# hrz2000/CustomNeRF

Hardware: AMD Instinct MI355X
Metric: training rays/s (higher is better)
Workload: dtype f16

## Files before the change

customnerf_amd/_lib.py:

```python
import ctypes as C
import os

import torch

_HERE = os.path.dirname(os.path.abspath(__file__))
LIB_PATH = os.path.join(_HERE, "libcustomnerf_hip.so")
ABI_VERSION = 7

vp, u32, u64, f32, i32 = C.c_void_p, C.c_uint32, C.c_uint64, C.c_float, C.c_int

SIGNATURES = {
    "cnerf_abi_version": [],
    "cnerf_profile_stage_events": [vp, u32],
    "cnerf_near_far_from_aabb": [vp, vp, vp, u32, f32, vp, vp, vp],
    "cnerf_sph_from_ray": [vp, vp, f32, u32, vp, vp],
    "cnerf_morton3D": [vp, u32, vp, vp],
    "cnerf_morton3D_invert": [vp, u32, vp, vp],
    "cnerf_packbits": [vp, u32, f32, vp, vp],
    "cnerf_march_rays_train": [vp, vp, vp, f32, f32, u32, u32, u32, u32, u32, vp, vp, vp, vp, vp, vp, vp, vp, vp],
    "cnerf_march_rays_train_count": [vp, vp, vp, f32, f32, u32, u32, u32, u32, vp, vp, vp, vp, vp, vp],
    "cnerf_march_rays_train_write": [vp, vp, vp, f32, f32, u32, u32, u32, u32, u32, vp, vp, vp, vp, vp, vp, vp, vp],
    "cnerf_march_rays_train_count_hits": [vp, vp, vp, f32, f32, u32, u32, u32, u32, vp, vp, vp, vp, vp, vp, vp],
    "cnerf_march_rays_train_write_hits": [vp, vp, f32, f32, u32, u32, u32, u32, u32, vp, vp, vp, vp, vp, vp, vp, vp],
    "cnerf_composite_rays_train_forward": [vp, vp, vp, vp, u32, u32, f32, vp, vp, vp, u32, vp],
# ... 9 lines not shown
    "cnerf_grid_encode_backward_prepared": [vp, vp, vp, vp, u32, u32, u32, u32, u32, f32, u32, u32, i32, u32, i32, vp, u64, vp],
    "cnerf_grid_encode_backward_workspace_bytes": [vp, u32, u32, u32, u32, u32, f32, u32, i32, vp],
    "cnerf_grid_encode_backward_needs_plan": [vp, u32, u32, u32, u32, u32, f32, u32, u32, i32, vp],
    "cnerf_grad_total_variation": [vp, vp, vp, vp, f32, u32, u32, u32, u32, f32, u32, u32, i32, vp],
    "cnerf_cast_f32_to_f16": [vp, vp, u64, vp],
    "cnerf_field_forward": [vp, vp, vp, u32, u32, u32, u32, u32, vp, vp, vp, vp, vp, i32, vp],
    "cnerf_field_forward_strided": [vp, vp, vp, u32, u32, u32, u32, u32, vp, vp, vp, vp, vp, i32, u32, vp],
    "cnerf_field_backward": [vp, vp, vp, u32, u32, u32, u32, u32, vp, vp, vp, vp, vp, vp, vp, vp, vp, vp, u64, i32, vp],
    "cnerf_field_backward_ex": [vp, vp, vp, u32, u32, u32, u32, u32, vp, vp, vp, vp, vp, vp, vp, vp, vp, vp, u64, i32, vp, vp],
    "cnerf_field_backward_workspace_bytes": [u32, u32, u32, u32, i32, vp],
    "cnerf_stream_capture_id": [vp, vp],
    "cnerf_field_weight_image_bytes": [u32, u32, u32, vp],
    "cnerf_field_pack_weights": [u32, u32, u32, vp, vp, vp, vp, u64, vp],
    "cnerf_field_forward_img": [vp, vp, vp, u32, u32, u32, u32, u32, vp, vp, vp, vp, vp, i32, u32, vp, vp],
    "cnerf_field_backward_img": [vp, vp, vp, u32, u32, u32, u32, u32, vp, vp, vp, vp, vp, vp, vp, vp, vp, vp, u64, i32, vp, vp, vp],
    "cnerf_mlp_forward": [vp, u32, vp, u32, u32, u32, u32, u32, i32, vp, u32, i32, vp],
    "cnerf_mlp_backward": [vp, u32, vp, vp, u32, u32, u32, u32, u32, u32, i32, vp, u32, vp, vp, u64, i32, vp],
    "cnerf_mlp_backward_workspace_bytes": [u32, u32, u32, u32, u32, i32, vp],
    "cnerf_generate_rays": [vp, u32, u32, u32, f32, f32, f32, f32, f32, i32, vp, vp, vp],
    "cnerf_generate_rays_fisheye": [vp, u32, u32, u32, f32, f32, f32, f32, f32, vp, vp, vp, vp],
    "cnerf_occupancy_points": [vp, u32, f32, f32, vp, vp],
    "cnerf_occupancy_update": [vp, u32, f32, vp, vp, vp],
    "cnerf_occupancy_finalize_pack": [vp, u32, f32, vp, u32, vp, vp, vp],
    "cnerf_sample_pdf": [vp, vp, vp, u32, u32, u32, vp, vp],
    "cnerf_sample_coarse": [vp, vp, vp, vp, vp, vp, u32, u32, vp, vp, vp],
    "cnerf_sample_fine_merge": [vp, vp, vp, vp, vp, vp, vp, vp, u32, u32, u32, vp, vp, vp],
    "cnerf_sample_fine_merge_split": [vp, vp, vp, vp, vp, vp, vp, vp, u32, u32, u32, vp, vp, vp, vp, vp],
    "cnerf_sample_coarse_unit": [vp, vp, vp, vp, vp, vp, u32, u32, vp, vp, vp, f32, vp],
    "cnerf_sample_fine_merge_split_unit": [vp, vp, vp, vp, vp, vp, vp, vp, u32, u32, u32, vp, vp, vp, vp, f32, vp],
    "cnerf_composite_run": [vp, vp, vp, vp, vp, u32, u32, u32, i32, f32, vp, vp, vp],
# ... 242 lines not shown
```

customnerf_amd/csrc/field_bwd.hip:

```cpp
#include "field_bwd_common.h"
#include "field_dw.h"

struct FieldWs {
    uint32_t enc, h1, h2, fea, hd, hr, dir, z1, z2, z3, zd, zdo, zr, zro, rows;
};
__host__ __device__ __forceinline__ FieldWs fb_ws_layout(const FieldDims &d) {
    FieldWs w;
    uint32_t o = 0;
    w.enc = o; o += d.enc_pad;
    w.h1 = o; o += 64;
    w.h2 = o; o += (d.n_hidden_geo == 2) ? 64 : 0;
    w.fea = o; o += 64;
    w.hd = o; o += 64;
    w.hr = o; o += 64;
    w.dir = o; o += 32;
    w.z1 = o; o += 64;
    w.z2 = o; o += (d.n_hidden_geo == 2) ? 64 : 0;
    w.z3 = o; o += 64;
    w.zd = o; o += 64;
    w.zdo = o; o += 8;
    w.zr = o; o += 64;
    w.zro = o; o += 8;
    w.rows = o;
    return w;
// ... 221 lines not shown
    fb_add_job(pl, wo.zro, dm.n_rgb_out, wo.hr, 64, 2, FLD_HID * in_r0, 64, 0, 16);
    const uint32_t splits = fb_dw_splits(n_tiles, pl.k_tiles_per_split);
    float *partials = reinterpret_cast<float *>(reinterpret_cast<unsigned char *>(workspace) + fb_part_off(dm, P_, H ? CNERF_F16 : CNERF_F32));
    hipLaunchKernelGGL((k_field_bwd_dw<H>), dim3(pl.n_tiles, splits), dim3(FLD_THREADS), 0, st, workspace, ld, n_tiles, pl, g_net, g_den, g_rgb, partials);
    rc = cn_launch_status();
    if (rc) return rc;
    ff_reduce_partials(partials, splits, po.total, po.d0, po.r0 - po.d0, g_net, g_den, g_rgb, st);
    return cn_launch_status();
}

static bool fb_use_fused(const FieldDims &dm, int dtype) {
    static const int env = cn_tune_env("CNERF_FIELD_FUSED_BWD", 1);
    return env && dtype == CNERF_F16 && dm.enc_pad <= 32;
}

extern "C" {

int cnerf_field_backward_workspace_bytes(uint32_t P_, uint32_t enc_dim, uint32_t n_hidden_geo, uint32_t n_rgb_out, int dtype, uint64_t *bytes) {
    if (!bytes) return CNERF_ENULL;
    FieldDims dm;
    int rc = fld_dims(enc_dim, n_hidden_geo, n_rgb_out, dm);
    if (rc) return rc;
    if (dtype != CNERF_F32 && dtype != CNERF_F16) return CNERF_EINVAL;
    if (fb_use_fused(dm, dtype)) *bytes = ff_workspace_bytes(dm);
    else *bytes = fb_workspace_bytes(dm, P_, dtype);
    return CNERF_OK;
}

int cnerf_field_backward(const void *enc, const float *xyz, const float *dirs, uint32_t dir_group, uint32_t P_, uint32_t enc_dim,
                         uint32_t n_hidden_geo, uint32_t n_rgb_out, const float *params_net, const float *params_den, const float *params_rgb,
                         const float *grad_sigma, const float *grad_rgbc, void *grad_enc, float *grad_params_net, float *grad_params_den,
// ... 3 lines not shown
}

int cnerf_field_backward_ex(const void *enc, const float *xyz, const float *dirs, uint32_t dir_group, uint32_t P_, uint32_t enc_dim,
                            uint32_t n_hidden_geo, uint32_t n_rgb_out, const float *params_net, const float *params_den, const float *params_rgb,
                            const float *grad_sigma, const float *grad_rgbc, void *grad_enc, float *grad_params_net, float *grad_params_den,
                            float *grad_params_rgb, void *workspace, uint64_t workspace_bytes, int dtype, const uint8_t *tile_live, void *stream) {
    return cnerf_field_backward_img(enc, xyz, dirs, dir_group, P_, enc_dim, n_hidden_geo, n_rgb_out, params_net, params_den, params_rgb, grad_sigma, grad_rgbc,
                                    grad_enc, grad_params_net, grad_params_den, grad_params_rgb, workspace, workspace_bytes, dtype, tile_live, nullptr, stream);
}

int cnerf_field_backward_img(const void *enc, const float *xyz, const float *dirs, uint32_t dir_group, uint32_t P_, uint32_t enc_dim,
                             uint32_t n_hidden_geo, uint32_t n_rgb_out, const float *params_net, const float *params_den, const float *params_rgb,
                             const float *grad_sigma, const float *grad_rgbc, void *grad_enc, float *grad_params_net, float *grad_params_den,
                             float *grad_params_rgb, void *workspace, uint64_t workspace_bytes, int dtype, const uint8_t *tile_live,
                             const void *weight_image, void *stream) {
    FieldDims dm;
    int rc = fld_dims(enc_dim, n_hidden_geo, n_rgb_out, dm);
    if (rc) return rc;
    if (dtype != CNERF_F32 && dtype != CNERF_F16) return CNERF_EINVAL;
    if (P_ == 0) return CNERF_OK;
    if (!enc || !xyz || !dirs || !params_net || !params_den || !params_rgb || !grad_sigma || !grad_rgbc || !grad_enc || !grad_params_net ||
        !grad_params_den || !grad_params_rgb || !workspace)
        return CNERF_ENULL;
    if (dir_group == 0 || (((uintptr_t)grad_rgbc) & 15) || (((uintptr_t)workspace) & 15) || (((uintptr_t)weight_image) & 15)) return CNERF_EINVAL;
    uint64_t need = 0;
    cnerf_field_backward_workspace_bytes(P_, enc_dim, n_hidden_geo, n_rgb_out, dtype, &need);
    if (workspace_bytes < need) return CNERF_EINVAL;
    if (fb_use_fused(dm, dtype))
        return ff_launch(enc, xyz, dirs, dir_group, P_, dm, params_net, params_den, params_rgb, grad_sigma, grad_rgbc, grad_enc, grad_params_net,
                         grad_params_den, grad_params_rgb, workspace, tile_live, CN_STREAM(stream), weight_image);
    if (dtype == CNERF_F16)
        return fb_launch<true>(enc, xyz, dirs, dir_group, P_, dm, params_net, params_den, params_rgb, grad_sigma, grad_rgbc, grad_enc,
                               grad_params_net, grad_params_den, grad_params_rgb, workspace, CN_STREAM(stream));
    return fb_launch<false>(enc, xyz, dirs, dir_group, P_, dm, params_net, params_den, params_rgb, grad_sigma, grad_rgbc, grad_enc, grad_params_net,
                            grad_params_den, grad_params_rgb, workspace, CN_STREAM(stream));
}

}
```

customnerf_amd/csrc/field_bwd_common.h:

```cpp
#pragma once
#include "field_common.h"


template <bool H, int T, int NS>
__device__ __forceinline__ void fb_gemm(const typename Prec<H>::elem_t *wf, uint32_t S, uint32_t s0, const typename Prec<H>::frag_t *b, uint32_t lane,
                                        cn_f16v (&acc)[T]) {
    asm volatile("" ::: "memory");
    fld_gemm<H, T, NS>(wf, S, s0, b, lane, acc);
}

template <bool H>
__device__ __forceinline__ void fb_stage_layer_T(typename Prec<H>::elem_t *dst, const float *__restrict__ W, uint32_t rows, uint32_t in_stride,
                                                 uint32_t col0, uint32_t n_in, uint32_t T, uint32_t S) {
    using P = Prec<H>;
    const uint32_t total = T * S * 64 * P::J;
    for (uint32_t i = threadIdx.x; i < total; i += blockDim.x) {
        const uint32_t j = i % P::J, lane = (i / P::J) % 64, ts = i / (P::J * 64);
        const uint32_t s = ts % S, t = ts / S;
        const uint32_t col = 32 * t + (lane & 31), hi = lane >> 5;
        const uint32_t row = (uint32_t)fld_col_clayout<H>(s, hi, j);
        float v = 0.0f;
        if (row < rows && col < n_in) v = W[(size_t)row * in_stride + col0 + col];
        dst[i] = (typename P::elem_t)v;
    }
// ... 139 lines not shown
    o.n1 = p; p += (dm.n_hidden_geo == 2) ? 4096 : 0;
    o.n2 = p; p += 4096;
    o.d0 = p; p += 4096;
    o.dO = p; p += 16 * 64;
    o.r0 = p; p += 64 * 96;
    o.rO = p; p += 16 * 64;
    o.total = p;
    return o;
}

void ff_reduce_partials(const float *partials, uint32_t n_partials, uint32_t total, uint32_t n_net, uint32_t n_den, float *g_net, float *g_den, float *g_rgb,
                        hipStream_t st);
uint64_t ff_workspace_bytes(const FieldDims &dm);
int ff_launch(const void *enc, const float *xyz, const float *dirs, uint32_t dir_group, uint32_t P_, const FieldDims &dm, const float *pnet,
              const float *pden, const float *prgb, const float *g_sigma, const float *g_rgbc, void *grad_enc, float *g_net, float *g_den,
              float *g_rgb, void *workspace, const uint8_t *tile_live, hipStream_t st, const void *wimg);
bool x2_eligible(const FieldDims &dm);
int x2_launch(const void *enc, const float *xyz, const float *dirs, uint32_t dir_group, uint32_t P_, const FieldDims &dm, const float *pnet, const float *pden,
              const float *prgb, const float *g_sigma, const float *g_rgbc, void *grad_enc, float *g_net, float *g_den, float *g_rgb, void *workspace,
              uint32_t max_partials, const uint8_t *tile_live, hipStream_t st, const void *wimg);
```

customnerf_amd/csrc/field_bwd_fused.hip:

```cpp
#include "field_bwd_common.h"

#define FF_ROWB 256
#define FF_ROWS 256
#define FF_STAGE_BYTES (FF_ROWB * FF_ROWS)
#define FF_PIN(col, hi) asm volatile("" : "+v"(col), "+v"(hi)::"memory")

__device__ __forceinline__ void ff_put(unsigned char *st, uint32_t row, uint32_t col, _Float16 v) {
    *reinterpret_cast<_Float16 *>(st + row * FF_ROWB + (((col >> 3) ^ (row & 15)) << 4) + ((col & 7) << 1)) = v;
}
__device__ __forceinline__ cn_h8 ff_frag(const unsigned char *st, uint32_t row, uint32_t s, uint32_t hi) {
    return *reinterpret_cast<const cn_h8 *>(st + row * FF_ROWB + ((((2 * s + hi)) ^ (row & 15)) << 4));
}
__device__ __forceinline__ void ff_stage_clayout(unsigned char *st, uint32_t row0, uint32_t col, uint32_t hi, const cn_h8 *b) {
#pragma unroll
    for (int s = 0; s < 4; s++) {
        asm volatile("" : "+v"(col), "+v"(hi)::"memory");
#pragma unroll
        for (int j = 0; j < 8; j++) ff_put(st, row0 + (uint32_t)fld_col_clayout<true>(s, hi, j), col, b[s][j]);
    }
}
template <int NS>
__device__ __forceinline__ void ff_stage_natural(unsigned char *st, uint32_t row0, uint32_t col, uint32_t hi, const cn_h8 *b) {
#pragma unroll
    for (int s = 0; s < NS; s++) {
// ... 300 lines not shown
        *dst = gn;
        if (!(fabsf(gn) <= 3.4e38f) && found_inf) *found_inf = 1.0f;
    }
}

#define FF_MAX_BLOCKS 512
uint64_t ff_workspace_bytes(const FieldDims &dm) { return (uint64_t)FF_MAX_BLOCKS * ff_offsets(dm).total * sizeof(float) + 256; }

void ff_reduce_partials(const float *partials, uint32_t n_partials, uint32_t total, uint32_t n_net, uint32_t n_den, float *g_net, float *g_den, float *g_rgb,
                        hipStream_t st) {
    hipLaunchKernelGGL(k_field_reduce_partials, dim3(cn_div_up(total, 64)), dim3(256), 0, st, partials, n_partials, total, n_net, n_den, g_net, g_den, g_rgb, g_cn_found_inf);
}

int ff_launch(const void *enc, const float *xyz, const float *dirs, uint32_t dir_group, uint32_t P_, const FieldDims &dm, const float *pnet,
              const float *pden, const float *prgb, const float *g_sigma, const float *g_rgbc, void *grad_enc, float *g_net, float *g_den,
              float *g_rgb, void *workspace, const uint8_t *tile_live, hipStream_t st, const void *wimg) {
    if (x2_eligible(dm)) {
        return x2_launch(enc, xyz, dirs, dir_group, P_, dm, pnet, pden, prgb, g_sigma, g_rgbc, grad_enc, g_net, g_den, g_rgb, workspace, FF_MAX_BLOCKS, tile_live, st,
                         wimg);
    }
    (void)wimg;
    const FieldLds lo = fld_lds_layout<true>(dm);
    const FieldLdsT lt = fb_ldsT_layout<true>(dm);
    const uint32_t lds_bytes = (lo.off[7] + lt.off[7]) * sizeof(_Float16) + FF_STAGE_BYTES;
    if (lds_bytes > 160 * 1024) return CNERF_EINVAL;
    const uint32_t n_tiles = cn_div_up(P_, FLD_TILE);
    uint32_t blocks = cn_div_up(n_tiles, FLD_WAVES);
    if (blocks > 256) blocks = 256;
    const FfOff po = ff_offsets(dm);
    float *partials = reinterpret_cast<float *>(workspace);
    hipError_t e = hipMemsetAsync(partials, 0, (size_t)blocks * po.total * sizeof(float), st);
    if (e != hipSuccess) return (int)e;
    const bool ok = fld_dispatch(dm, [&](auto se16, auto ng) {
        auto kern = k_field_bwd_fused<se16, ng, (se16 + 1) / 2>;
        (void)hipFuncSetAttribute(reinterpret_cast<const void *>(kern), hipFuncAttributeMaxDynamicSharedMemorySize, lds_bytes);
        hipLaunchKernelGGL(kern, dim3(blocks), dim3(FLD_THREADS), lds_bytes, st, enc, xyz, dirs, dir_group, P_, dm, pnet, pden, prgb, g_sigma, g_rgbc, grad_enc,
// ... 9 lines not shown
```

customnerf_amd/csrc/field_bwd_x2.hip:

```cpp
#include "field_bwd_common.h"

typedef short x4_s4 __attribute__((__vector_size__(4 * sizeof(short))));
typedef short x4_s2 __attribute__((ext_vector_type(2)));

#define X4_K 1024

struct X4Img { uint32_t c0, c1; };
__device__ __forceinline__ uint32_t x4_img_swz(uint32_t byte_off) { return byte_off ^ (((byte_off >> 9) & 3u) << 6); }
template <int S>
__device__ __forceinline__ cn_h8 x4_frag_T(const unsigned char *layer, X4Img lane_off, int tp, int sp) {
    const uint32_t c = ((sp >> 1) * S + 2 * tp) * 1024 + (16 * (sp & 1)) * 16;
    union { cn_h8 h; x4_s4 s[2]; } f;
    f.s[0] = __builtin_amdgcn_ds_read_tr16_b64_v4i16((x4_s4 __attribute__((address_space(3))) *)(layer + lane_off.c0 + c));
    f.s[1] = __builtin_amdgcn_ds_read_tr16_b64_v4i16((x4_s4 __attribute__((address_space(3))) *)(layer + lane_off.c1 + c));
    return f.h;
}
__device__ __forceinline__ X4Img x4_lane_off_w(uint32_t l, bool natural_cols) {
    const uint32_t G = l >> 4, i = l & 15, rho = i >> 2, q = i & 3;
    const uint32_t hi = natural_cols ? (q >> 1) : (q & 1), j0 = natural_cols ? 4 * (q & 1) : 4 * (q >> 1);
    const uint32_t base = (G & 1) * 1024 + hi * 512 + (4 * (l >> 5) + rho) * 16;
    X4Img o;
    o.c0 = x4_img_swz(base) + j0 * 2;
    o.c1 = x4_img_swz(base + 8 * 16) + j0 * 2;
    return o;
// ... 38 lines not shown

template <int T, int NS, int S>
__device__ __forceinline__ void x4_frags_T(const unsigned char *layer, X4Img lane_off, cn_h8 (&w)[NS][T]) {
#pragma unroll
    for (int s = 0; s < NS; s++) {
#pragma unroll
        for (int t = 0; t < T; t++) w[s][t] = x4_frag_T<S>(layer, lane_off, t, s);
    }
}
template <int T, int NS>
__device__ __forceinline__ void x4_gemm_pre(const cn_h8 (&w)[NS][T], const cn_h8 *b, cn_f16v (&acc)[T]) {
#pragma unroll
    for (int s = 0; s < NS; s++) {
#pragma unroll
        for (int t = 0; t < T; t++) acc[t] = Prec<true>::mfma(w[s][t], b[s], acc[t]);
    }
}
__device__ __forceinline__ void x4_pin() { __builtin_amdgcn_sched_barrier(0); }

__device__ __forceinline__ uint32_t x4_cvt_pk(float a, float b) {
    const cn_h2 v = {(_Float16)a, (_Float16)b};
    return __builtin_bit_cast(uint32_t, v);
}
__device__ __forceinline__ uint32_t x4_pk_relu(uint32_t v) {
    uint32_t r;
    asm("v_pk_max_i16 %0, %1, 0" : "=v"(r) : "v"(v));
    return r;
}
__device__ __forceinline__ uint32_t x4_pk_posmask(uint32_t act) {
    uint32_t t, m;
// ... 101 lines not shown
#define X2_A_X0 0
#define X2_A_H1 (2 * X4_K)
#define X2_A_H2 (6 * X4_K)
#define X2_A_Z2 (10 * X4_K)
#define X2_A_Z1 (14 * X4_K)
#define X2_B (X2_A + 18 * X4_K)
#define X2_B_HD 0
#define X2_B_HR (4 * X4_K)
#define X2_B_DIR (8 * X4_K)
#define X2_B_ZR (10 * X4_K)
#define X2_B_ZD (14 * X4_K)
#define X2_B_BRO (18 * X4_K)
#define X2_B_BDO (20 * X4_K)
#define X2_PAIR_BYTES (X2_B + 22 * X4_K)

template <int NGEO, bool SKIP>
__global__ void __launch_bounds__(FLD_THREADS) k_field_bwd_x2(const void *__restrict__ enc, const float *__restrict__ xyz, const float *__restrict__ dirs,
                                                              uint32_t dir_group, uint32_t P_, FieldDims dm, const float *__restrict__ pnet,
                                                              const float *__restrict__ pden, const float *__restrict__ prgb,
                                                              const float *__restrict__ g_sigma, const float *__restrict__ g_rgbc,
                                                              void *__restrict__ grad_enc, float *__restrict__ partials, uint32_t ablate_arg,
                                                              const uint8_t *__restrict__ tile_live, const void *__restrict__ wimg) {
#ifdef CNERF_TUNING
    const uint32_t ablate = ablate_arg;
#else
    constexpr uint32_t ablate = 0;
    (void)ablate_arg;
#endif
    constexpr bool H = true;
    constexpr int SENC = 2;
    using PR = Prec<H>;
    using frag_t = typename PR::frag_t;
    using elem_t = typename PR::elem_t;
    __shared__ __attribute__((aligned(16))) elem_t x2_w[FLD_HID * (32 + 3 * FLD_HID + (FLD_HID + FLD_DIR)) + 2 * 32 * FLD_HID];
    extern __shared__ __attribute__((aligned(16))) unsigned char fld_lds[];
    elem_t *wl = x2_w;
    const FieldLds lo = fld_lds_layout<H>(dm);
// ... 215 lines not shown
            x4_store(part, po.n0, dm.enc_pad, 0, 64, dm.enc_pad, a, 0, li, hi, wn0[a]);
#pragma unroll
            for (int b = 0; b < 2; b++) {
                x4_store(part, po.n2, 64, 0, 64, 64, a, b, li, hi, wn2[a][b]);
                if (NGEO == 2) x4_store(part, po.n1, 64, 0, 64, 64, a, b, li, hi, wn1[a][b]);
            }
        }
    } else {
        cn_f16v wro[2], wrd[2], wrf[2][2], wdo[2], wd0[2][2];
#pragma unroll
        for (int a = 0; a < 2; a++) {
            x4_zero(wro[a]); x4_zero(wrd[a]); x4_zero(wdo[a]);
#pragma unroll
            for (int b = 0; b < 2; b++) { x4_zero(wrf[a][b]); x4_zero(wd0[a][b]); }
        }
        struct BIn { float x, y, z, gs, dx, dy, dz; float4 gc; uint32_t tile; };
        auto load_in = [&](uint32_t window) __attribute__((always_inline)) {
            BIn r;
            r.tile = window == END ? END : tile_at(window);
            const uint32_t p = min((window == END ? 0u : r.tile) * FLD_TILE + li, P_ - 1);
            r.x = xyz[(size_t)p * 3]; r.y = xyz[(size_t)p * 3 + 1]; r.z = xyz[(size_t)p * 3 + 2];
            r.gs = g_sigma[p];
            r.gc = *reinterpret_cast<const float4 *>(g_rgbc + (size_t)p * 4);
            const float *dp = dirs + (size_t)(p / dir_group) * 3;
            r.dx = dp[0]; r.dy = dp[1]; r.dz = dp[2];
            return r;
        };
        LiveIt it;
        it.base = 0; it.m = pair_mask(0, false);
        uint32_t pk = it_next(it, false);
        uint32_t kend = pk == END ? 0u : END;
        BIn I0 = load_in(pk), I1 = I0;
        unsigned char *my = xch + X2_B;
        const bool dir_uniform = (dir_group % FLD_TILE) == 0;
        auto phase = [&](uint32_t k, const BIn &cur, BIn &nxt) __attribute__((always_inline)) {
            X4_T0();
            asm volatile("" ::: "memory");
            if (k >= 1) {
                if (pk != END) pk = it_next(it, false);
                if (pk == END && kend == END) kend = k;
                nxt = load_in(pk);
            }
            if (k >= 1 && !(ablate & 4) && cur.tile < n_tiles) {
                const uint32_t i = k - 1;
                const uint32_t tile = cur.tile;
                const bool valid = tile * FLD_TILE + li < P_;
                const unsigned char *fe = xch + X2_FEA + (i & 1) * 4 * X4_K;
                frag_t fea[4], dfr[SDIR];
                x4_fetch<4>(fe, lane, fea);
                if (dir_uniform) fld_dir_frags_uniform(cur.dx, cur.dy, cur.dz, lane, hi, my + X2_B_ZD, dfr);
                else fld_dir_frags_from<H>(cur.dx, cur.dy, cur.dz, valid, hi, dfr);
                x4_publish<SDIR>(my + X2_B_DIR, lane, dfr);
                cn_f16v acc[2], out[1];
                frag_t hd[4], hr[4];
                fld_zero(acc);
                x4_gemm<2, S64>(wl + lo.off[3], S64, 0, fea, lane, acc);
                x4_c_to_b<true>(acc, hd);
                x4_publish<4>(my + X2_B_HD, lane, hd);
                fld_zero(out);
                x4_gemm<1, S64>(wl + lo.off[4], S64, 0, hd, lane, out);
                const float raw = (float)(_Float16)out[0][0];
                fld_zero(acc);
                x4_gemm<2, S64>(wl + lo.off[5], SR0, 0, fea, lane, acc);
                x4_gemm<2, SDIR>(wl + lo.off[5], SR0, S64, dfr, lane, acc);
                x4_c_to_b<true>(acc, hr);
                x4_publish<4>(my + X2_B_HR, lane, hr);
                fld_zero(out);
                x4_gemm<1, S64>(wl + lo.off[6], S64, 0, hr, lane, out);
                frag_t bro[1], bdo[1];
                {
                    cn_h8 f = PR::zero(), g = PR::zero();
                    if (valid && hi == 0) {
                        const float x = cur.x, y = cur.y, z = cur.z;
                        const float gg = 5.0f * __expf(-(x * x + y * y + z * z) * (1.0f / 0.08f));
                        g[0] = (_Float16)(cur.gs * __expf(fminf(fmaxf(raw + gg, -15.0f), 15.0f)));
                        const float gcv[4] = {cur.gc.x, cur.gc.y, cur.gc.z, cur.gc.w};
#pragma unroll
                        for (int k = 0; k < 4; k++) {
                            const float sg = (float)(_Float16)__builtin_amdgcn_rcpf(1.0f + __expf(-out[0][k]));
                            f[k] = (_Float16)((k < (int)dm.n_rgb_out) ? gcv[k] * sg * (1.0f - sg) : 0.0f);
                        }
                    }
                    bro[0] = f; bdo[0] = g;
                }
                x4_publish<1>(my + X2_B_BRO, lane, bro);
                x4_publish<1>(my + X2_B_BDO, lane, bdo);
                cn_f16v dfea[2];
                fld_zero(dfea);
                cn_h8 fa[2][2];
                cn_h8 wh[S64][2];
                cn_h8 zo[2], z[2][2], a[2][2], d[2];
                fld_zero(acc);
                x4_gemm_T<2, 1, S64>(wb + off_rO, lw, bro, acc);
                x4_frags_T<2, S64, SR0>(wb + off_r0, lw, wh);
// ... 61 lines not shown
#ifdef CNERF_TUNING
    if ((ablate & 32) && lane == 0) {
        unsigned long long *tt = reinterpret_cast<unsigned long long *>(partials + (size_t)510 * po.total) + ((size_t)blockIdx.x * 4 + wave) * 2;
        tt[0] = tw_; tt[1] = tb_;
    }
#endif
}

bool x2_eligible(const FieldDims &dm) {
    static const int on = cn_tune_env("CNERF_FIELD_X2_BWD", 1);
    return on && dm.enc_pad == 32 && (dm.n_hidden_geo == 1 || dm.n_hidden_geo == 2);
}

int x2_launch(const void *enc, const float *xyz, const float *dirs, uint32_t dir_group, uint32_t P_, const FieldDims &dm, const float *pnet, const float *pden,
              const float *prgb, const float *g_sigma, const float *g_rgbc, void *grad_enc, float *g_net, float *g_den, float *g_rgb, void *workspace,
              uint32_t max_partials, const uint8_t *tile_live, hipStream_t st, const void *wimg) {
    const FieldLds lo = fld_lds_layout<true>(dm);
    if (lo.off[7] > FLD_HID * (32 + 3 * FLD_HID + (FLD_HID + FLD_DIR)) + 2 * 32 * FLD_HID) return CNERF_EINVAL;
    const uint32_t lds_bytes = 2 * X2_PAIR_BYTES;
    const uint32_t n_tiles = cn_div_up(P_, FLD_TILE);
    uint32_t blocks = cn_div_up(n_tiles, 2);
    if (blocks > max_partials / 2) blocks = max_partials / 2;
    if (blocks > 256) blocks = 256;
    const FfOff po = ff_offsets(dm);
    float *partials = reinterpret_cast<float *>(workspace);
    static const int ablate = cn_tune_env("CNERF_X2_ABLATE", 0);
    if ((ablate & 32) && blocks > 255) blocks = 255;
#define X2_LAUNCH(KERN)                                                                                                                    \
    {                                                                                                                                      \
        auto kern = KERN;                                                                                                                  \
        (void)hipFuncSetAttribute(reinterpret_cast<const void *>(kern), hipFuncAttributeMaxDynamicSharedMemorySize, lds_bytes);            \
        hipLaunchKernelGGL(kern, dim3(blocks), dim3(FLD_THREADS), lds_bytes, st, enc, xyz, dirs, dir_group, P_, dm, pnet, pden, prgb, g_sigma, g_rgbc, \
                           grad_enc, partials, (uint32_t)ablate, tile_live, wimg);                                                             \
    }
    cn_stage(4, st);
    if (tile_live) {
        if (dm.n_hidden_geo == 2) X2_LAUNCH((k_field_bwd_x2<2, true>)) else X2_LAUNCH((k_field_bwd_x2<1, true>))
    } else {
        if (dm.n_hidden_geo == 2) X2_LAUNCH((k_field_bwd_x2<2, false>)) else X2_LAUNCH((k_field_bwd_x2<1, false>))
    }
    cn_stage(5, st);
    int rc = cn_launch_status();
    if (rc) return rc;
    ff_reduce_partials(partials, blocks * 2, po.total, po.d0, po.r0 - po.d0, g_net, g_den, g_rgb, st);
    cn_stage(6, st);
    return cn_launch_status();
}
```

customnerf_amd/field.py:

```python
import torch
from torch.autograd import Function

from ._lib import lib, check, ptr, stream, F16, F32, require_cuda, scratch_key, grad_chain_wait, grad_chain_record, query_u64, ScratchCache


def capture_id():
    return query_u64(lib.cnerf_stream_capture_id, stream())


def packed_weights(cache, enc_dim, n_hidden_geo, n_rgb_out, p_net, p_den, p_rgb):
    require_cuda(p_net, p_den, p_rgb)
    key = tuple((p.data_ptr(), p._version, getattr(p, '_cnerf_epoch', 0)) for p in (p_net, p_den, p_rgb))
    slot = (scratch_key(p_net.device), enc_dim, n_hidden_geo, n_rgb_out)
    ent = cache.get(slot)
    if ent is None:
        need = query_u64(lib.cnerf_field_weight_image_bytes, int(enc_dim), int(n_hidden_geo), int(n_rgb_out))
        ent = cache[slot] = {'img': torch.empty(need, dtype=torch.uint8, device=p_net.device), 'key': None, 'cap': 0, 'cap_key': None}
    cap = capture_id()
    if cap:
        fresh = ent['cap'] == cap and ent['cap_key'] == key
        ent['cap'], ent['cap_key'], ent['key'] = cap, key, None
    else:
        fresh = ent['key'] == key
        ent['key'] = key
# ... 19 lines not shown

def field_forward_rows(enc, row0, xyz_rows, dirs, dir_group, enc_dim, n_hidden_geo, n_rgb_out, p_net, p_den, p_rgb, sigma_out, rgbc_out, wimg=None):
    require_cuda(enc, xyz_rows, dirs, p_net, p_den, p_rgb, sigma_out, rgbc_out, wimg)
    n = xyz_rows.shape[0]
    assert enc.is_contiguous() and row0 + n <= enc.shape[1] and xyz_rows.is_contiguous() and dirs.is_contiguous()
    assert sigma_out.is_contiguous() and rgbc_out.is_contiguous() and sigma_out.numel() == n and rgbc_out.numel() == 4 * n
    dt = F16 if enc.dtype == torch.float16 else F32
    src = enc.data_ptr() + row0 * enc.shape[2] * enc.element_size()
    check(lib.cnerf_field_forward_img(src, ptr(xyz_rows), ptr(dirs), int(dir_group), n, int(enc_dim), int(n_hidden_geo), int(n_rgb_out),
                                      ptr(p_net), ptr(p_den), ptr(p_rgb), ptr(sigma_out), ptr(rgbc_out), dt, int(enc.shape[1]), ptr(wimg), stream()),
          "field_forward")


_WS = ScratchCache(factor=1.1, pad=256)


def _workspace(P, enc_dim, n_hidden_geo, n_rgb_out, dt, device):
    need = query_u64(lib.cnerf_field_backward_workspace_bytes, P, enc_dim, n_hidden_geo, n_rgb_out, dt)
    return _WS.reserve(scratch_key(device), need, device)


class FieldFunction(Function):

    @staticmethod
    def forward(ctx, enc, xyz, dirs, dir_group, enc_dim, n_hidden_geo, n_rgb_out, p_net, p_den, p_rgb, grad_in_place=False, wimg=None):
        ctx.params = (p_net, p_den, p_rgb) if grad_in_place else None
        ctx.wimg = wimg
        xyz = xyz.contiguous().float()
        dirs = dirs.contiguous().float()
        sigma, rgbc = field_forward_raw(enc, xyz, dirs, dir_group, enc_dim, n_hidden_geo, n_rgb_out, p_net, p_den, p_rgb, True, wimg)
        ctx.save_for_backward(enc, xyz, dirs, p_net, p_den, p_rgb)
        ctx.cfg = (dir_group, enc_dim, n_hidden_geo, n_rgb_out)
        return sigma, rgbc

    @staticmethod
    def backward(ctx, g_sigma, g_rgbc):
        enc, xyz, dirs, p_net, p_den, p_rgb = ctx.saved_tensors
        dir_group, enc_dim, n_hidden_geo, n_rgb_out = ctx.cfg
        P = xyz.shape[0]
        dt = F16 if enc.dtype == torch.float16 else F32
        tile_live = None
        flags = getattr(g_sigma, '_cnerf_tile_live', None)
        if flags is not None:
            tl, ps, vs, pc, vc = flags
            if (g_sigma.data_ptr() == ps and g_sigma._version == vs and g_rgbc.data_ptr() == pc and g_rgbc._version == vc and g_sigma.is_contiguous()
                    and g_rgbc.is_contiguous() and g_sigma.dtype == torch.float32 and g_rgbc.dtype == torch.float32 and tl.numel() * 32 == P and tl.is_cuda):
                tile_live = tl
        g_sigma = g_sigma.contiguous().float()
        g_rgbc = g_rgbc.contiguous().float()
        g_enc = torch.empty_like(enc)
        in_place = ctx.params is not None and all(p.grad is not None and p.grad.dtype == torch.float32 and p.grad.is_contiguous() and
                                                  p.grad.device == p.device for p in ctx.params)
        if in_place:
            g_net, g_den, g_rgb = (p.grad for p in ctx.params)
        else:
            g_all = torch.zeros(p_net.numel() + p_den.numel() + p_rgb.numel(), dtype=torch.float32, device=p_net.device)
            g_net, g_den, g_rgb = (t.view_as(p) for t, p in zip(g_all.split([p_net.numel(), p_den.numel(), p_rgb.numel()]), (p_net, p_den, p_rgb)))
        ws = _workspace(P, enc_dim, n_hidden_geo, n_rgb_out, dt, xyz.device)
        if in_place:
            grad_chain_wait(xyz.device)
        check(lib.cnerf_field_backward_img(ptr(enc), ptr(xyz), ptr(dirs), int(dir_group), P, int(enc_dim), int(n_hidden_geo), int(n_rgb_out),
                                           ptr(p_net), ptr(p_den), ptr(p_rgb), ptr(g_sigma), ptr(g_rgbc), ptr(g_enc), ptr(g_net), ptr(g_den), ptr(g_rgb),
                                           ptr(ws), ws.numel(), dt, ptr(tile_live), ptr(getattr(ctx, 'wimg', None)), stream()), "field_backward")
        if in_place:
            grad_chain_record(xyz.device)
            return g_enc, None, None, None, None, None, None, None, None, None, None, None
        return g_enc, None, None, None, None, None, None, g_net, g_den, g_rgb, None, None


class FieldAttach(Function):

    @staticmethod
    def forward(ctx, enc, xyz, dirs, dir_group, enc_dim, n_hidden_geo, n_rgb_out, p_net, p_den, p_rgb, grad_in_place, sigma, rgbc, wimg=None):
        ctx.params = (p_net, p_den, p_rgb) if grad_in_place else None
        ctx.wimg = wimg
        ctx.save_for_backward(enc, xyz.contiguous().float(), dirs.contiguous().float(), p_net, p_den, p_rgb)
        ctx.cfg = (dir_group, enc_dim, n_hidden_geo, n_rgb_out)
        return sigma.detach(), rgbc.detach()

    @staticmethod
    def backward(ctx, g_sigma, g_rgbc):
        return FieldFunction.backward(ctx, g_sigma, g_rgbc)[:11] + (None, None, None)


def field_attach(enc, xyz, dirs, dir_group, enc_dim, n_hidden_geo, n_rgb_out, p_net, p_den, p_rgb, sigma, rgbc, grad_in_place=False, wimg=None):
    return FieldAttach.apply(enc, xyz, dirs, dir_group, enc_dim, n_hidden_geo, n_rgb_out, p_net, p_den, p_rgb, grad_in_place, sigma, rgbc, wimg)


def field(enc, xyz, dirs, dir_group, enc_dim, n_hidden_geo, n_rgb_out, p_net, p_den, p_rgb, grad_in_place=False, wimg=None):
    return FieldFunction.apply(enc, xyz, dirs, dir_group, enc_dim, n_hidden_geo, n_rgb_out, p_net, p_den, p_rgb, grad_in_place, wimg)
```

include/customnerf_hip.h:

```cpp
#ifndef CUSTOMNERF_HIP_H
#define CUSTOMNERF_HIP_H

#include <stdint.h>

#ifdef __cplusplus
extern "C" {
#endif

#define CNERF_OK 0
#define CNERF_EINVAL (-1)
#define CNERF_ENULL (-2)

#define CNERF_F32 0
#define CNERF_F16 1

#define CNERF_ABI_VERSION 7
int cnerf_abi_version(void);
const char *cnerf_target_arch(void);
#define CNERF_STAGE_EVENTS 8
int cnerf_profile_stage_events(void *const *events, uint32_t n);


int cnerf_near_far_from_aabb(const float *rays_o, const float *rays_d, const float *aabb, uint32_t N,
                             float min_near, float *nears, float *fars, void *stream);
// ... 118 lines not shown
int cnerf_grid_backward_adam_consumed(int *yes);

int cnerf_stream_capture_id(void *stream, uint64_t *id);
int cnerf_field_weight_image_bytes(uint32_t enc_dim, uint32_t n_hidden_geo, uint32_t n_rgb_out, uint64_t *bytes);
int cnerf_field_pack_weights(uint32_t enc_dim, uint32_t n_hidden_geo, uint32_t n_rgb_out, const float *params_net, const float *params_den,
                             const float *params_rgb, void *image, uint64_t image_bytes, void *stream);
int cnerf_field_forward_img(const void *enc, const float *xyz, const float *dirs, uint32_t dir_group, uint32_t P, uint32_t enc_dim,
                            uint32_t n_hidden_geo, uint32_t n_rgb_out, const float *params_net, const float *params_den,
                            const float *params_rgb, float *sigma, float *rgbc, int dtype, uint32_t enc_level_stride,
                            const void *weight_image, void *stream);
int cnerf_field_backward_img(const void *enc, const float *xyz, const float *dirs, uint32_t dir_group, uint32_t P, uint32_t enc_dim,
                             uint32_t n_hidden_geo, uint32_t n_rgb_out, const float *params_net, const float *params_den,
                             const float *params_rgb, const float *grad_sigma, const float *grad_rgbc, void *grad_enc,
                             float *grad_params_net, float *grad_params_den, float *grad_params_rgb, void *workspace,
                             uint64_t workspace_bytes, int dtype, const uint8_t *tile_live, const void *weight_image, void *stream);

int cnerf_mlp_forward(const void *x, uint32_t ldx, const float *params, uint32_t P, uint32_t n_in, uint32_t n_out,
                      uint32_t n_neurons, uint32_t n_hidden_layers, int output_activation, void *y, uint32_t ldy, int dtype,
                      void *stream);
int cnerf_mlp_backward(const void *x, uint32_t ldx, const float *params, const void *grad_y, uint32_t ldgy, uint32_t P,
                       uint32_t n_in, uint32_t n_out, uint32_t n_neurons, uint32_t n_hidden_layers, int output_activation,
                       void *grad_x, uint32_t ldgx, float *grad_params, void *workspace, uint64_t workspace_bytes, int dtype,
                       void *stream);
int cnerf_mlp_backward_workspace_bytes(uint32_t P, uint32_t n_in, uint32_t n_out, uint32_t n_neurons,
                                       uint32_t n_hidden_layers, int dtype, uint64_t *bytes);

int cnerf_generate_rays(const float *c2w, uint32_t V, uint32_t H, uint32_t W, float fx, float fy, float cx, float cy,
                        float level, int convention, float *origins, float *directions, void *stream);
int cnerf_generate_rays_fisheye(const float *c2w, uint32_t V, uint32_t H, uint32_t W, float fx, float fy, float cx, float cy,
                                float level, const float *distortion_host, float *origins, float *directions, void *stream);
// ... 204 lines not shown
```

Before: 8.399 million.

## Reuse saved forward sigma/rgb in fused field backward instead of recomputing heads

Saves the forward sigma and rgbc outputs and passes them to the fused x2 backward kernel through a new arming call. The kernel reads the activated outputs directly to form the sigma-exp and sigmoid derivatives, skipping the density and RGB output GEMMs and the Gaussian density bias recompute. It also preloads the weight fragments ahead of the hidden-layer GEMMs. In exchange it reads two extra per-point buffers, holds them in memory until backward, and relies on clamping the saved sigma to match the forward exp clamp, which may differ slightly in f16 rounding.

Result: no change. 8.460 million (median of 6 runs) (+0.7%).

```diff
diff --git a/customnerf_amd/_lib.py b/customnerf_amd/_lib.py
--- a/customnerf_amd/_lib.py
+++ b/customnerf_amd/_lib.py
@@ -47,6 +47,7 @@
     "cnerf_field_pack_weights": [u32, u32, u32, vp, vp, vp, vp, u64, vp],
     "cnerf_field_forward_img": [vp, vp, vp, u32, u32, u32, u32, u32, vp, vp, vp, vp, vp, i32, u32, vp, vp],
     "cnerf_field_backward_img": [vp, vp, vp, u32, u32, u32, u32, u32, vp, vp, vp, vp, vp, vp, vp, vp, vp, vp, u64, i32, vp, vp, vp],
+    "cnerf_field_backward_outputs": [vp, vp, u32],
     "cnerf_mlp_forward": [vp, u32, vp, u32, u32, u32, u32, u32, i32, vp, u32, i32, vp],
     "cnerf_mlp_backward": [vp, u32, vp, vp, u32, u32, u32, u32, u32, u32, i32, vp, u32, vp, vp, u64, i32, vp],
     "cnerf_mlp_backward_workspace_bytes": [u32, u32, u32, u32, u32, i32, vp],
diff --git a/customnerf_amd/csrc/field_bwd.hip b/customnerf_amd/csrc/field_bwd.hip
--- a/customnerf_amd/csrc/field_bwd.hip
+++ b/customnerf_amd/csrc/field_bwd.hip
@@ -259,7 +259,18 @@
     return env && dtype == CNERF_F16 && dm.enc_pad <= 32;
 }
 
+static struct { const float *sigma, *rgbc; uint32_t P; } g_fb_outputs = {nullptr, nullptr, 0};
+
 extern "C" {
+
+int cnerf_field_backward_outputs(const float *sigma, const float *rgbc, uint32_t P_) {
+    g_fb_outputs = {nullptr, nullptr, 0};
+    if (!sigma && !rgbc) return CNERF_OK;
+    if (!sigma || !rgbc) return CNERF_ENULL;
+    if ((((uintptr_t)sigma) & 3) || (((uintptr_t)rgbc) & 15) || P_ == 0) return CNERF_EINVAL;
+    g_fb_outputs = {sigma, rgbc, P_};
+    return CNERF_OK;
+}
 
 int cnerf_field_backward_workspace_bytes(uint32_t P_, uint32_t enc_dim, uint32_t n_hidden_geo, uint32_t n_rgb_out, int dtype, uint64_t *bytes) {
     if (!bytes) return CNERF_ENULL;
@@ -293,6 +304,8 @@
                              const float *grad_sigma, const float *grad_rgbc, void *grad_enc, float *grad_params_net, float *grad_params_den,
                              float *grad_params_rgb, void *workspace, uint64_t workspace_bytes, int dtype, const uint8_t *tile_live,
                              const void *weight_image, void *stream) {
+    const auto armed = g_fb_outputs;
+    g_fb_outputs = {nullptr, nullptr, 0};
     FieldDims dm;
     int rc = fld_dims(enc_dim, n_hidden_geo, n_rgb_out, dm);
     if (rc) return rc;
@@ -305,9 +318,12 @@
     uint64_t need = 0;
     cnerf_field_backward_workspace_bytes(P_, enc_dim, n_hidden_geo, n_rgb_out, dtype, &need);
     if (workspace_bytes < need) return CNERF_EINVAL;
-    if (fb_use_fused(dm, dtype))
+    if (fb_use_fused(dm, dtype)) {
+        const bool reuse = armed.sigma && armed.P == P_ && x2_eligible(dm);
         return ff_launch(enc, xyz, dirs, dir_group, P_, dm, params_net, params_den, params_rgb, grad_sigma, grad_rgbc, grad_enc, grad_params_net,
-                         grad_params_den, grad_params_rgb, workspace, tile_live, CN_STREAM(stream), weight_image);
+                         grad_params_den, grad_params_rgb, workspace, tile_live, CN_STREAM(stream), weight_image, reuse ? armed.sigma : nullptr,
+                         reuse ? armed.rgbc : nullptr);
+    }
     if (dtype == CNERF_F16)
         return fb_launch<true>(enc, xyz, dirs, dir_group, P_, dm, params_net, params_den, params_rgb, grad_sigma, grad_rgbc, grad_enc,
                                grad_params_net, grad_params_den, grad_params_rgb, workspace, CN_STREAM(stream));
diff --git a/customnerf_amd/csrc/field_bwd_common.h b/customnerf_amd/csrc/field_bwd_common.h
--- a/customnerf_amd/csrc/field_bwd_common.h
+++ b/customnerf_amd/csrc/field_bwd_common.h
@@ -177,8 +177,8 @@
 uint64_t ff_workspace_bytes(const FieldDims &dm);
 int ff_launch(const void *enc, const float *xyz, const float *dirs, uint32_t dir_group, uint32_t P_, const FieldDims &dm, const float *pnet,
               const float *pden, const float *prgb, const float *g_sigma, const float *g_rgbc, void *grad_enc, float *g_net, float *g_den,
-              float *g_rgb, void *workspace, const uint8_t *tile_live, hipStream_t st, const void *wimg);
+              float *g_rgb, void *workspace, const uint8_t *tile_live, hipStream_t st, const void *wimg, const float *fwd_sigma, const float *fwd_rgbc);
 bool x2_eligible(const FieldDims &dm);
 int x2_launch(const void *enc, const float *xyz, const float *dirs, uint32_t dir_group, uint32_t P_, const FieldDims &dm, const float *pnet, const float *pden,
               const float *prgb, const float *g_sigma, const float *g_rgbc, void *grad_enc, float *g_net, float *g_den, float *g_rgb, void *workspace,
-              uint32_t max_partials, const uint8_t *tile_live, hipStream_t st, const void *wimg);
+              uint32_t max_partials, const uint8_t *tile_live, hipStream_t st, const void *wimg, const float *fwd_sigma, const float *fwd_rgbc);
diff --git a/customnerf_amd/csrc/field_bwd_fused.hip b/customnerf_amd/csrc/field_bwd_fused.hip
--- a/customnerf_amd/csrc/field_bwd_fused.hip
+++ b/customnerf_amd/csrc/field_bwd_fused.hip
@@ -338,12 +338,12 @@
 
 int ff_launch(const void *enc, const float *xyz, const float *dirs, uint32_t dir_group, uint32_t P_, const FieldDims &dm, const float *pnet,
               const float *pden, const float *prgb, const float *g_sigma, const float *g_rgbc, void *grad_enc, float *g_net, float *g_den,
-              float *g_rgb, void *workspace, const uint8_t *tile_live, hipStream_t st, const void *wimg) {
+              float *g_rgb, void *workspace, const uint8_t *tile_live, hipStream_t st, const void *wimg, const float *fwd_sigma, const float *fwd_rgbc) {
     if (x2_eligible(dm)) {
         return x2_launch(enc, xyz, dirs, dir_group, P_, dm, pnet, pden, prgb, g_sigma, g_rgbc, grad_enc, g_net, g_den, g_rgb, workspace, FF_MAX_BLOCKS, tile_live, st,
-                         wimg);
-    }
-    (void)wimg;
+                         wimg, fwd_sigma, fwd_rgbc);
+    }
+    (void)wimg; (void)fwd_sigma; (void)fwd_rgbc;
     const FieldLds lo = fld_lds_layout<true>(dm);
     const FieldLdsT lt = fb_ldsT_layout<true>(dm);
     const uint32_t lds_bytes = (lo.off[7] + lt.off[7]) * sizeof(_Float16) + FF_STAGE_BYTES;
diff --git a/customnerf_amd/csrc/field_bwd_x2.hip b/customnerf_amd/csrc/field_bwd_x2.hip
--- a/customnerf_amd/csrc/field_bwd_x2.hip
+++ b/customnerf_amd/csrc/field_bwd_x2.hip
@@ -76,6 +76,14 @@
     for (int s = 0; s < NS; s++) {
 #pragma unroll
         for (int t = 0; t < T; t++) acc[t] = Prec<true>::mfma(w[s][t], b[s], acc[t]);
+    }
+}
+template <int T, int NS>
+__device__ __forceinline__ void x4_frags_fwd(const _Float16 *wf, uint32_t S, uint32_t s0, uint32_t lane, cn_h8 (&w)[NS][T]) {
+#pragma unroll
+    for (int s = 0; s < NS; s++) {
+#pragma unroll
+        for (int t = 0; t < T; t++) w[s][t] = x4_load_frag(wf, t, S, s0 + s, lane);
     }
 }
 __device__ __forceinline__ void x4_pin() { __builtin_amdgcn_sched_barrier(0); }
@@ -207,13 +215,14 @@
 #define X2_B_BDO (20 * X4_K)
 #define X2_PAIR_BYTES (X2_B + 22 * X4_K)
 
-template <int NGEO, bool SKIP>
+template <int NGEO, bool SKIP, bool REUSE = false>
 __global__ void __launch_bounds__(FLD_THREADS) k_field_bwd_x2(const void *__restrict__ enc, const float *__restrict__ xyz, const float *__restrict__ dirs,
                                                               uint32_t dir_group, uint32_t P_, FieldDims dm, const float *__restrict__ pnet,
                                                               const float *__restrict__ pden, const float *__restrict__ prgb,
                                                               const float *__restrict__ g_sigma, const float *__restrict__ g_rgbc,
                                                               void *__restrict__ grad_enc, float *__restrict__ partials, uint32_t ablate_arg,
-                                                              const uint8_t *__restrict__ tile_live, const void *__restrict__ wimg) {
+                                                              const uint8_t *__restrict__ tile_live, const void *__restrict__ wimg,
+                                                              const float *__restrict__ fwd_sigma, const float *__restrict__ fwd_rgbc) {
 #ifdef CNERF_TUNING
     const uint32_t ablate = ablate_arg;
 #else
@@ -459,12 +468,19 @@
 #pragma unroll
             for (int b = 0; b < 2; b++) { x4_zero(wrf[a][b]); x4_zero(wd0[a][b]); }
         }
-        struct BIn { float x, y, z, gs, dx, dy, dz; float4 gc; uint32_t tile; };
+        struct BIn { float x, y, z, gs, dx, dy, dz, fs; float4 gc, fc; uint32_t tile; };
         auto load_in = [&](uint32_t window) __attribute__((always_inline)) {
             BIn r;
             r.tile = window == END ? END : tile_at(window);
             const uint32_t p = min((window == END ? 0u : r.tile) * FLD_TILE + li, P_ - 1);
-            r.x = xyz[(size_t)p * 3]; r.y = xyz[(size_t)p * 3 + 1]; r.z = xyz[(size_t)p * 3 + 2];
+            if constexpr (REUSE) {
+                r.x = r.y = r.z = 0.0f;
+                r.fs = fwd_sigma[p];
+                r.fc = *reinterpret_cast<const float4 *>(fwd_rgbc + (size_t)p * 4);
+            } else {
+                r.x = xyz[(size_t)p * 3]; r.y = xyz[(size_t)p * 3 + 1]; r.z = xyz[(size_t)p * 3 + 2];
+                r.fs = 0.0f; r.fc = make_float4(0.0f, 0.0f, 0.0f, 0.0f);
+            }
             r.gs = g_sigma[p];
             r.gc = *reinterpret_cast<const float4 *>(g_rgbc + (size_t)p * 4);
             const float *dp = dirs + (size_t)(p / dir_group) * 3;
@@ -478,6 +494,13 @@
         BIn I0 = load_in(pk), I1 = I0;
         unsigned char *my = xch + X2_B;
         const bool dir_uniform = (dir_group % FLD_TILE) == 0;
+        [[maybe_unused]] float e_lo = 0.0f, e_hi = 0.0f;
+        if constexpr (REUSE) {
+            float a_lo = -15.0f, a_hi = 15.0f;
+            asm volatile("" : "+v"(a_lo), "+v"(a_hi));
+            e_lo = __builtin_bit_cast(float, __builtin_amdgcn_readfirstlane(__builtin_bit_cast(int, __expf(a_lo))));
+            e_hi = __builtin_bit_cast(float, __builtin_amdgcn_readfirstlane(__builtin_bit_cast(int, __expf(a_hi))));
+        }
         auto phase = [&](uint32_t k, const BIn &cur, BIn &nxt) __attribute__((always_inline)) {
             X4_T0();
             asm volatile("" ::: "memory");
@@ -496,33 +519,64 @@
                 if (dir_uniform) fld_dir_frags_uniform(cur.dx, cur.dy, cur.dz, lane, hi, my + X2_B_ZD, dfr);
                 else fld_dir_frags_from<H>(cur.dx, cur.dy, cur.dz, valid, hi, dfr);
                 x4_publish<SDIR>(my + X2_B_DIR, lane, dfr);
-                cn_f16v acc[2], out[1];
+                cn_f16v acc[2];
+                [[maybe_unused]] cn_f16v out[1];
                 frag_t hd[4], hr[4];
                 fld_zero(acc);
-                x4_gemm<2, S64>(wl + lo.off[3], S64, 0, fea, lane, acc);
+                if constexpr (REUSE) {
+                    cn_h8 wf[S64][2];
+                    x4_frags_fwd<2, S64>(wl + lo.off[3], S64, 0, lane, wf);
+                    x4_pin();
+                    x4_gemm_pre<2, S64>(wf, fea, acc);
+                } else {
+                    x4_gemm<2, S64>(wl + lo.off[3], S64, 0, fea, lane, acc);
+                }
                 x4_c_to_b<true>(acc, hd);
                 x4_publish<4>(my + X2_B_HD, lane, hd);
-                fld_zero(out);
-                x4_gemm<1, S64>(wl + lo.off[4], S64, 0, hd, lane, out);
-                const float raw = (float)(_Float16)out[0][0];
+                float raw = 0.0f;
+                if constexpr (!REUSE) {
+                    fld_zero(out);
+                    x4_gemm<1, S64>(wl + lo.off[4], S64, 0, hd, lane, out);
+                    raw = (float)(_Float16)out[0][0];
+                }
                 fld_zero(acc);
-                x4_gemm<2, S64>(wl + lo.off[5], SR0, 0, fea, lane, acc);
-                x4_gemm<2, SDIR>(wl + lo.off[5], SR0, S64, dfr, lane, acc);
+                if constexpr (REUSE) {
+                    cn_h8 wf[S64][2], wd[SDIR][2];
+                    x4_frags_fwd<2, S64>(wl + lo.off[5], SR0, 0, lane, wf);
+                    x4_frags_fwd<2, SDIR>(wl + lo.off[5], SR0, S64, lane, wd);
+                    x4_pin();
+                    x4_gemm_pre<2, S64>(wf, fea, acc);
+                    x4_gemm_pre<2, SDIR>(wd, dfr, acc);
+                } else {
+                    x4_gemm<2, S64>(wl + lo.off[5], SR0, 0, fea, lane, acc);
+                    x4_gemm<2, SDIR>(wl + lo.off[5], SR0, S64, dfr, lane, acc);
+                }
                 x4_c_to_b<true>(acc, hr);
                 x4_publish<4>(my + X2_B_HR, lane, hr);
-                fld_zero(out);
-                x4_gemm<1, S64>(wl + lo.off[6], S64, 0, hr, lane, out);
+                if constexpr (!REUSE) {
+                    fld_zero(out);
+                    x4_gemm<1, S64>(wl + lo.off[6], S64, 0, hr, lane, out);
+                }
                 frag_t bro[1], bdo[1];
                 {
                     cn_h8 f = PR::zero(), g = PR::zero();
                     if (valid && hi == 0) {
-                        const float x = cur.x, y = cur.y, z = cur.z;
-                        const float gg = 5.0f * __expf(-(x * x + y * y + z * z) * (1.0f / 0.08f));
-                        g[0] = (_Float16)(cur.gs * __expf(fminf(fmaxf(raw + gg, -15.0f), 15.0f)));
+                        float ex;
+                        if constexpr (REUSE) {
+                            ex = fminf(fmaxf(cur.fs, e_lo), e_hi);
+                        } else {
+                            const float x = cur.x, y = cur.y, z = cur.z;
+                            const float gg = 5.0f * __expf(-(x * x + y * y + z * z) * (1.0f / 0.08f));
+                            ex = __expf(fminf(fmaxf(raw + gg, -15.0f), 15.0f));
+                        }
+                        g[0] = (_Float16)(cur.gs * ex);
                         const float gcv[4] = {cur.gc.x, cur.gc.y, cur.gc.z, cur.gc.w};
+                        [[maybe_unused]] const float fcv[4] = {cur.fc.x, cur.fc.y, cur.fc.z, cur.fc.w};
 #pragma unroll
                         for (int k = 0; k < 4; k++) {
-                            const float sg = (float)(_Float16)__builtin_amdgcn_rcpf(1.0f + __expf(-out[0][k]));
+                            float sg;
+                            if constexpr (REUSE) sg = fcv[k];
+                            else sg = (float)(_Float16)__builtin_amdgcn_rcpf(1.0f + __expf(-out[0][k]));
                             f[k] = (_Float16)((k < (int)dm.n_rgb_out) ? gcv[k] * sg * (1.0f - sg) : 0.0f);
                         }
                     }
@@ -614,7 +668,7 @@
 
 int x2_launch(const void *enc, const float *xyz, const float *dirs, uint32_t dir_group, uint32_t P_, const FieldDims &dm, const float *pnet, const float *pden,
               const float *prgb, const float *g_sigma, const float *g_rgbc, void *grad_enc, float *g_net, float *g_den, float *g_rgb, void *workspace,
-              uint32_t max_partials, const uint8_t *tile_live, hipStream_t st, const void *wimg) {
+              uint32_t max_partials, const uint8_t *tile_live, hipStream_t st, const void *wimg, const float *fwd_sigma, const float *fwd_rgbc) {
     const FieldLds lo = fld_lds_layout<true>(dm);
     if (lo.off[7] > FLD_HID * (32 + 3 * FLD_HID + (FLD_HID + FLD_DIR)) + 2 * 32 * FLD_HID) return CNERF_EINVAL;
     const uint32_t lds_bytes = 2 * X2_PAIR_BYTES;
@@ -631,10 +685,16 @@
         auto kern = KERN;                                                                                                                  \
         (void)hipFuncSetAttribute(reinterpret_cast<const void *>(kern), hipFuncAttributeMaxDynamicSharedMemorySize, lds_bytes);            \
         hipLaunchKernelGGL(kern, dim3(blocks), dim3(FLD_THREADS), lds_bytes, st, enc, xyz, dirs, dir_group, P_, dm, pnet, pden, prgb, g_sigma, g_rgbc, \
-                           grad_enc, partials, (uint32_t)ablate, tile_live, wimg);                                                             \
+                           grad_enc, partials, (uint32_t)ablate, tile_live, wimg, fwd_sigma, fwd_rgbc);                                        \
     }
     cn_stage(4, st);
-    if (tile_live) {
+    if (fwd_sigma && fwd_rgbc) {
+        if (tile_live) {
+            if (dm.n_hidden_geo == 2) X2_LAUNCH((k_field_bwd_x2<2, true, true>)) else X2_LAUNCH((k_field_bwd_x2<1, true, true>))
+        } else {
+            if (dm.n_hidden_geo == 2) X2_LAUNCH((k_field_bwd_x2<2, false, true>)) else X2_LAUNCH((k_field_bwd_x2<1, false, true>))
+        }
+    } else if (tile_live) {
         if (dm.n_hidden_geo == 2) X2_LAUNCH((k_field_bwd_x2<2, true>)) else X2_LAUNCH((k_field_bwd_x2<1, true>))
     } else {
         if (dm.n_hidden_geo == 2) X2_LAUNCH((k_field_bwd_x2<2, false>)) else X2_LAUNCH((k_field_bwd_x2<1, false>))
diff --git a/customnerf_amd/field.py b/customnerf_amd/field.py
--- a/customnerf_amd/field.py
+++ b/customnerf_amd/field.py
@@ -57,6 +57,8 @@
 
 _WS = ScratchCache(factor=1.1, pad=256)
 
+REUSE_FORWARD_OUTPUTS = True
+
 
 def _workspace(P, enc_dim, n_hidden_geo, n_rgb_out, dt, device):
     need = query_u64(lib.cnerf_field_backward_workspace_bytes, P, enc_dim, n_hidden_geo, n_rgb_out, dt)
@@ -72,13 +74,13 @@
         xyz = xyz.contiguous().float()
         dirs = dirs.contiguous().float()
         sigma, rgbc = field_forward_raw(enc, xyz, dirs, dir_group, enc_dim, n_hidden_geo, n_rgb_out, p_net, p_den, p_rgb, True, wimg)
-        ctx.save_for_backward(enc, xyz, dirs, p_net, p_den, p_rgb)
+        ctx.save_for_backward(enc, xyz, dirs, p_net, p_den, p_rgb, sigma, rgbc)
         ctx.cfg = (dir_group, enc_dim, n_hidden_geo, n_rgb_out)
         return sigma, rgbc
 
     @staticmethod
     def backward(ctx, g_sigma, g_rgbc):
-        enc, xyz, dirs, p_net, p_den, p_rgb = ctx.saved_tensors
+        enc, xyz, dirs, p_net, p_den, p_rgb, sigma, rgbc = ctx.saved_tensors
         dir_group, enc_dim, n_hidden_geo, n_rgb_out = ctx.cfg
         P = xyz.shape[0]
         dt = F16 if enc.dtype == torch.float16 else F32
@@ -102,6 +104,9 @@
         ws = _workspace(P, enc_dim, n_hidden_geo, n_rgb_out, dt, xyz.device)
         if in_place:
             grad_chain_wait(xyz.device)
+        if (REUSE_FORWARD_OUTPUTS and dt == F16 and sigma.dtype == torch.float32 and rgbc.dtype == torch.float32 and sigma.is_contiguous()
+                and rgbc.is_contiguous() and sigma.numel() == P and rgbc.numel() == 4 * P and rgbc.data_ptr() % 16 == 0):
+            check(lib.cnerf_field_backward_outputs(ptr(sigma), ptr(rgbc), P), "field_backward_outputs")
         check(lib.cnerf_field_backward_img(ptr(enc), ptr(xyz), ptr(dirs), int(dir_group), P, int(enc_dim), int(n_hidden_geo), int(n_rgb_out),
                                            ptr(p_net), ptr(p_den), ptr(p_rgb), ptr(g_sigma), ptr(g_rgbc), ptr(g_enc), ptr(g_net), ptr(g_den), ptr(g_rgb),
                                            ptr(ws), ws.numel(), dt, ptr(tile_live), ptr(getattr(ctx, 'wimg', None)), stream()), "field_backward")
@@ -117,7 +122,7 @@
     def forward(ctx, enc, xyz, dirs, dir_group, enc_dim, n_hidden_geo, n_rgb_out, p_net, p_den, p_rgb, grad_in_place, sigma, rgbc, wimg=None):
         ctx.params = (p_net, p_den, p_rgb) if grad_in_place else None
         ctx.wimg = wimg
-        ctx.save_for_backward(enc, xyz.contiguous().float(), dirs.contiguous().float(), p_net, p_den, p_rgb)
+        ctx.save_for_backward(enc, xyz.contiguous().float(), dirs.contiguous().float(), p_net, p_den, p_rgb, sigma, rgbc)
         ctx.cfg = (dir_group, enc_dim, n_hidden_geo, n_rgb_out)
         return sigma.detach(), rgbc.detach()
 
diff --git a/include/customnerf_hip.h b/include/customnerf_hip.h
--- a/include/customnerf_hip.h
+++ b/include/customnerf_hip.h
@@ -156,6 +156,7 @@
                              const float *params_rgb, const float *grad_sigma, const float *grad_rgbc, void *grad_enc,
                              float *grad_params_net, float *grad_params_den, float *grad_params_rgb, void *workspace,
                              uint64_t workspace_bytes, int dtype, const uint8_t *tile_live, const void *weight_image, void *stream);
+int cnerf_field_backward_outputs(const float *sigma, const float *rgbc, uint32_t P);
 
 int cnerf_mlp_forward(const void *x, uint32_t ldx, const float *params, uint32_t P, uint32_t n_in, uint32_t n_out,
                       uint32_t n_neurons, uint32_t n_hidden_layers, int output_activation, void *y, uint32_t ldy, int dtype,
```
